# hazdzz/STGCN

Measured on AMD Instinct MI355X. Metric: training windows/sec, METR-LA ChebConv K=3 bs=32, higher is better.
Workload: dtype f32; 1 GPU; C2: METR-LA 207 nodes, STGCNChebGraphConv Ks=3 Kt=3, n_his=12, bs=32 per GPU, fp32, dropout 0.5, AdamW lr 1e-3 wd 1e-3; full step zero_grad+fwd+MSE+bwd+opt; graph=real metr_la adj -> sym_norm_lap -> cheb GSO, global_batch=32, parallelism=dp1, output_block=fused HIP path (stgcn_outblock_*), launch=hipGraph replay, chains=1, backward_products=fp32, operator_products=fp32

## Files before the change

stgcn_amd/csrc/stgcn_capi_bwd.inc:

```

namespace {
int launch_hook_rowstats(const stgcn_ln_hook* hook, const float* dx, long slabs, hipStream_t st) {
    LnBwdArgs hl = zeroed<LnBwdArgs>();
    const LnRowstatOut o = rowstat_out(hook);
    hl.dy = dx; hl.y = o.y; hl.beta = o.beta; hl.gamma = o.gamma; hl.rowstat = o.rowstat;
    hl.n = o.N * o.C; hl.N = o.N; hl.C = o.C; hl.act = o.act; hl.training = o.training; hl.slabs = slabs;
    hl.keep_scale = o.keep_scale; hl.thresh = o.thresh; hl.seed = o.seed; hl.offset = o.offset; hl.offset_dev = o.offset_dev;
    STGCN_LAUNCH_ET("ln_bwd_rowstats", st, (ln_bwd_rowstats_kernel<ET>), dim3(cdiv(hl.slabs * (hl.n / 4), kThreads)), dim3(kThreads), 0, hl);
    return STGCN_OK;
}

struct BlockBwdCall : BlockCall {
    const float* gso_t_pad;
    const float* dy;
    const float* y;
    float* dx;
    const stgcn_ln_hook* dx_hook;
    LnBwdArgs ln;

    int launch_ln_bwd_stats() {
        ln = zeroed<LnBwdArgs>();
        ln.dy = dy; ln.y = y; ln.beta = P->ln_b; ln.U = saved + pl.sv_U2; ln.S = saved + pl.sv_S2; ln.gamma = P->ln_w;
        ln.mean = saved + pl.sv_mean; ln.rstd = saved + pl.sv_rstd; ln.rowstat = reinterpret_cast<float2*>(ws + pl.ws_rowstat_b);
        ln.dZ = ws + pl.ws_dZ2; ln.dgam_part = part() + r.bg.off_ln_g; ln.dbet_part = part() + r.bg.off_ln_b;
        ln.n = d->N * d->c2; ln.N = d->N; ln.C = d->c2; ln.act = d->act; ln.training = training(); ln.spg = r.bg.ln_spg; ln.slabs = r.slabs2;
        ln.keep_scale = keep_scale(); ln.thresh = drop_thresh(d->droprate); ln.seed = seed; ln.offset = offset; ln.offset_dev = offset_dev;
        if (!d->dy_rowstats_ready)
            STGCN_LAUNCH_ET("ln_bwd_rowstats", st, (ln_bwd_rowstats_kernel<ET>), dim3(cdiv(r.slabs2 * (ln.n / 4), kThreads)), dim3(kThreads), 0, ln);
        if (cdiv(ln.n / 4, kThreads) >= kLnBigColgroups) {
            ln.slabconst = reinterpret_cast<float2*>(ws + pl.ws_rowstat_b + 2 * r.rows2);
            STGCN_LAUNCH("ln_slab_consts", st, ln_slab_consts_kernel, dim3((unsigned)r.slabs2), dim3(kThreads), 64, ln);
        }
        return STGCN_OK;
    }
    int launch_ln_gate_bwd() {
        const BwdGeom& bg = r.bg;
        STGCN_LAUNCH("ln_gate_bwd", st, (ln_gate_bwd_kernel<float>), dim3(cdiv(ln.n / 4, kThreads), bg.ln_sg), dim3(kThreads),
                     (8 + 2 * bg.ln_spg) * sizeof(float), ln);
        return STGCN_OK;
    }
    int launch_tc2_bwd() {
        if (g_debug_stages && !g_bf16) {
            const int rc = launch_ln_gate_bwd();
            if (rc) return rc;
        }
        Tc2BwdArgs a = zeroed<Tc2BwdArgs>();
        a.y = hook_mask_from_y() ? y : nullptr;
        a.dy = dy; a.U = ln.U; a.S = ln.S; a.Wp = ws + pl.ws_W2p; a.bias = ws + pl.ws_b2; a.gamma = ln.gamma; a.mean = ln.mean; a.rstd = ln.rstd;
        a.rowstat = ln.rowstat; a.slabconst = ln.slabconst; a.G = saved + pl.sv_G; a.Wd = ws + pl.ws_W2dense; a.dYg = ws + pl.ws_dYg;
        a.part = part() + r.bg.off_k1; a.dgam_part = ln.dgam_part; a.dbet_part = ln.dbet_part;
        a.B = d->B; a.T1 = r.T1; a.T2 = r.T2; a.N = d->N; a.act = d->act; a.training = ln.training; a.node_tiles = r.bg.node_tiles;
        a.keep_scale = ln.keep_scale; a.thresh = ln.thresh; a.seed = seed; a.offset = offset; a.offset_dev = offset_dev;
        const bool recomp = r.tc2_bwd_recompute;
        const int training = ln.training;
        const size_t lds = r.tc2_bwd_lds;
        const dim3 grid((unsigned)r.bg.k1_wgs), blk(512);
#define STGCN_TC2_BWD(C2_, KT_)                                                                                        \
        do {                                                                                                               \
            if (training && d->act == STGCN_ACT_GLU) STGCN_LAUNCH_ETB("tc2_bwd", st, (tc2_bwd_kernel<C2_, KT_, true, 0, RC_, ET>), grid, blk, lds, a);   \
            else if (training) STGCN_LAUNCH_ETB("tc2_bwd", st, (tc2_bwd_kernel<C2_, KT_, true, 1, RC_, ET>), grid, blk, lds, a);      \
            else if (d->act == STGCN_ACT_GLU) STGCN_LAUNCH_ETB("tc2_bwd", st, (tc2_bwd_kernel<C2_, KT_, false, 0, RC_, ET>), grid, blk, lds, a);       \
            else STGCN_LAUNCH_ETB("tc2_bwd", st, (tc2_bwd_kernel<C2_, KT_, false, 1, RC_, ET>), grid, blk, lds, a);                 \
        } while (0)
#define STGCN_TC2_BWD_RC(C2_, KT_) do { if (recomp) { constexpr bool RC_ = true; STGCN_TC2_BWD(C2_, KT_); } else { constexpr bool RC_ = false; STGCN_TC2_BWD(C2_, KT_); } } while (0)
        if (d->Kt == 2) STGCN_TC2_BWD_RC(64, 2); else if (d->Kt == 3) STGCN_TC2_BWD_RC(64, 3); else STGCN_TC2_BWD_RC(64, 4);
#undef STGCN_TC2_BWD_RC
#undef STGCN_TC2_BWD
        return STGCN_OK;
    }
    int launch_staged_tc2_bwd() {
        STGCN_F32_ONLY("ln_gate_bwd + row-tile weight / data gradients of tmp_conv2");
        int rc = launch_ln_gate_bwd();
        if (rc) return rc;
        TconvBwdWeightArgs wa = zeroed<TconvBwdWeightArgs>();
        wa.ts = make_taps(saved + pl.sv_G, d->c1, d->Kt, d->N, r.T1, r.T2, 1, r.rows2);
        wa.dZ = ws + pl.ws_dZ2; wa.part = part() + r.bg.w2.off; wa.NC = r.NC2; wa.Mpad = r.bg.w2.Mpad; wa.rows_per_chunk = r.bg.w2.rows_per_chunk;
        wa.chunks = r.bg.w2.chunks;
        rc = launch_bwd_weight("tconv_bwd_weight.tc2", wa, r.bg.w2, st);
        if (rc) return rc;
        TconvBwdDataArgs a = zeroed<TconvBwdDataArgs>();
        a.ts = make_taps(ws + pl.ws_dZ2, r.NC2, d->Kt, d->N, r.T2, r.T1, -1, r.rows1);
        a.Wp = ws + pl.ws_W2d; a.KCH = d->Kt * r.NC2 / 16; a.Cin = d->c1; a.Gmask = saved + pl.sv_G; a.dX = ws + pl.ws_dYg;
        return launch_bwd_data("tconv_bwd_data.tc2", a, r.CP1 / 16, st);
    }
    int launch_block_gconv_bwd() {
        GconvBwdArgs a = zeroed<GconvBwdArgs>();
        a.dY = ws + pl.ws_dYg; a.X0 = saved + pl.sv_A; a.Xk = saved + pl.sv_Xk; a.LTp = gso_t_pad; a.W = P->gc_w;
        a.dA = ws + pl.ws_dA; a.part = part() + r.bg.off_gc; a.N = d->N; a.NP = r.NP; a.Ks = r.terms;
        a.kipf = d->graph_conv == STGCN_GC_KIPF; a.slabs = r.slabs1;
        a.Gk = r.tiled_gc ? ws + pl.ws_Gk : nullptr; a.tiles_per_wg = r.bg.gc_tiles_per_wg; a.wgs = r.bg.gc_count;
        a.XT = r.tiled_gc && r.terms > 1 ? ws + pl.ws_XT : nullptr;
        return launch_gconv_bwd(a, r.tiled_gc, st);
    }
    int launch_align_gate_bwd() {
        STGCN_F32_ONLY("align_gate_bwd");
        AlignBwdArgs a = zeroed<AlignBwdArgs>();
        a.dA = ws + pl.ws_dA; a.WaT = ws + pl.ws_WaT; a.dZ = ws + pl.ws_dZ1;
        if (r.recompute_tc1) {
            a.Wd = ws + pl.ws_W1dense; a.bias = ws + pl.ws_b1; a.KPd = r.KP1;
            a.ts = input_taps();
        } else {
            a.U = saved + pl.sv_U1; a.S = saved + pl.sv_S1;
        }
        a.part = part() + r.bg.off_al; a.rows = r.rows1; a.c0 = d->c0; a.c1 = d->c1; a.KCH = r.CP1 / 16; a.act = d->act;
        const size_t lds = (size_t)(64 * (d->c1 + 4) + 64 * (d->c0 + 4) + 16 * d->c1) * sizeof(float);
        if (d->c0 == 64) STGCN_LAUNCH("align_gate_bwd", st, (align_gate_bwd_kernel<1>), dim3(r.bg.al_wgs), dim3(kThreads), lds, a);
        else STGCN_LAUNCH("align_gate_bwd", st, (align_gate_bwd_kernel<2>), dim3(r.bg.al_wgs), dim3(kThreads), lds, a);
        return STGCN_OK;
    }
    int launch_tc1_bwd() {
        if (g_debug_stages && !g_bf16) {
            const int rc = launch_align_gate_bwd();
            if (rc) return rc;
        }
        Tc1BwdArgs a = zeroed<Tc1BwdArgs>();
        a.dA = ws + pl.ws_dA; a.U = saved + pl.sv_U1; a.S = saved + pl.sv_S1; a.x = x; a.WaD = ws + pl.ws_WaDense; a.Wd = ws + pl.ws_W1dense;
        a.dx = dx; a.part = part() + r.bg.off_k3; a.B = d->B; a.T = d->T; a.T1 = r.T1; a.N = d->N; a.node_tiles = r.bg.node_tiles;
        const bool hooked = dx_hook && dx_hook->rowstat, epi = hooked && dx_hook->C == d->c_in && dx_hook->N == d->N;
        if (epi) a.rs = rowstat_out(dx_hook);
        const bool x6 = r.tc1_bwd_x6;
        const size_t lds = r.tc1_bwd_lds;
        const dim3 grid((unsigned)r.bg.k3_wgs), blk(768);
#define STGCN_TC1_BWD(CIN_)                                                                                    \
        do {                                                                                                       \
            if (x6 && d->act == STGCN_ACT_GLU) STGCN_LAUNCH("tc1_bwd", st, (tc1_bwd_x6_kernel<64, CIN_, 3, 0>), grid, blk, lds, a);   \
            else if (x6) STGCN_LAUNCH("tc1_bwd", st, (tc1_bwd_x6_kernel<64, CIN_, 3, 1>), grid, blk, lds, a);             \
            else if (d->act == STGCN_ACT_GLU) STGCN_LAUNCH_ETB("tc1_bwd", st, (tc1_bwd_kernel<64, CIN_, 3, 0, ET>), grid, blk, lds, a);   \
            else STGCN_LAUNCH_ETB("tc1_bwd", st, (tc1_bwd_kernel<64, CIN_, 3, 1, ET>), grid, blk, lds, a);             \
        } while (0)
        if (d->c_in == 64) STGCN_TC1_BWD(64); else if (d->c_in == 32) STGCN_TC1_BWD(32); else STGCN_TC1_BWD(16);
#undef STGCN_TC1_BWD
        if (hooked && !epi) return launch_hook_rowstats(dx_hook, dx, (long)d->B * d->T, st);
        return STGCN_OK;
    }
    int launch_thin_bwd() {
        ThinBwdArgs a = zeroed<ThinBwdArgs>();
        a.dA = ws + pl.ws_dA; a.Wd = ws + pl.ws_W1dense; a.bias = ws + pl.ws_b1; a.WaT = ws + pl.ws_WaT;
        a.dZ = d->need_dx ? ws + pl.ws_dZ1 : nullptr; a.part = part() + r.bg.off_al; a.rows = r.rows1; a.c0 = d->c0; a.act = d->act;
        a.ts = input_taps();
        const dim3 grid(r.bg.al_wgs), blk(kThreads);
        if (!r.thin_bwd_waves) {
            const size_t lds = (size_t)(64 * 20 + 64 * (d->c0 + 4) + 64 * (2 * d->c0 + 4) + 64 * 20 + 256) * sizeof(float);
            STGCN_LAUNCH_ETB("align_gate_bwd", st, (thin_tc1_bwd_kernel<ET>), grid, blk, lds, a);
        } else if (d->act == STGCN_ACT_GLU) STGCN_LAUNCH_ETB("align_gate_bwd", st, (thin_tc1_bwd2_kernel<ET, 0>), grid, blk, thin_bwd2_lds_bytes(), a);
        else STGCN_LAUNCH_ETB("align_gate_bwd", st, (thin_tc1_bwd2_kernel<ET, 1>), grid, blk, thin_bwd2_lds_bytes(), a);
        return STGCN_OK;
    }
    int launch_tc1_bwd_weight() {
// ... 63 lines not shown
```

stgcn_amd/csrc/stgcn_kernels_tstep.hip.h:

```cpp
#pragma once
#include <type_traits>
#include "stgcn_device.hip.h"
#include "stgcn_kernels_fwd.hip.h"

namespace stgcn {

struct Tc2BwdArgs {
    const float* y;
    const float* dy;
    const float* U;
    const float* S;
    const float* Wp;
    const float* bias;
    const float* gamma;
    const float* mean;
    const float* rstd;
    const float2* rowstat;
    const float2* slabconst;
    const float* G;
    const float* Wd;
    float* dYg;
    float* part;
    float* dgam_part;
    float* dbet_part;
    int B, T1, T2, N, act, training, node_tiles;
    float keep_scale;
    uint32_t thresh;
    uint64_t seed, offset;
    const uint64_t* offset_dev;
};

constexpr int kTsMaxT = 32;
inline size_t tc2_bwd_lds_bytes(int C2, int Kt, int T1, int T2, bool recomp = true) {
    return ((size_t)(Kt + 1) * 16 * (2 * C2 + 4) + (size_t)T1 * 16 * 20 + 2 * 4 * 16 * 20 + 4 * (size_t)T2 + (recomp ? 2 * 16 * (2 * C2 + 4) : 0)) * sizeof(float);
}

template <int C2, int KT, bool TRAINING, int ACT, bool RECOMP, typename ET>
__global__ __launch_bounds__(512, (C2 == 64 && KT == 3 && ACT == 0 && !RECOMP) ? 4 : 1) void tc2_bwd_kernel(Tc2BwdArgs a) {
    typedef Mma<ET> MM;
    const ET* const dy_ = et_ptr<ET>(a.dy);
    const ET* const ym_ = et_ptr<ET>(a.y ? a.y : a.dy);
    const bool mask_y = TRAINING && a.y != nullptr;
    const ET* const U_ = et_ptr<ET>(a.U);
    const ET* const S_ = et_ptr<ET>(a.S);
    const ET* const G_ = et_ptr<ET>(a.G);
    ET* const dYg_ = et_ptr<ET>(a.dYg);
    constexpr int NC = 2 * C2, LDZ = NC + 4, NTW = NC / 64, QW = NC / 64, IT = C2 / 64, LDG = 20, RING = KT + 1, RED = 4 * 16 * LDG;
    extern __shared__ float stgcn_smem[];
    float* const Zt = stgcn_smem;
    float* const GT = Zt + RING * 16 * LDZ;
    float* const red = GT + a.T1 * 16 * LDG;
    float* const cs = red + 2 * RED;
    float* const USt = cs + 4 * a.T2;
    const bool roleE = threadIdx.x < 256;
    const int tid = threadIdx.x & 255, w = tid >> 6, lane = tid & 63, g = lane >> 4, l15 = lane & 15;
    const int N = a.N, T1 = a.T1, T2 = a.T2;
    const int r = tid >> 4, cq = tid & 15;
    const long items = (long)a.B * a.node_tiles;
    const long it_lo = items * (long)blockIdx.x / (long)gridDim.x, it_hi = items * ((long)blockIdx.x + 1) / (long)gridDim.x;
    float* const part = a.part + (size_t)blockIdx.x * (KT * 16 * NC + NC);
    STGCN_PHASE(8, 0);

    if (roleE) {
        struct Tile { Raw4<ET> dy[IT], u[IT], s[IT], y[IT]; };
        f32x4 dbu[IT], dbq[IT];
#pragma unroll
        for (int it = 0; it < IT; ++it) { dbu[it] = zero4(); dbq[it] = zero4(); }
        const uint64_t off = a.offset + (a.offset_dev ? *a.offset_dev : 0);
        const uint64_t n4 = ((uint64_t)N * C2) >> 2;
        for (long item = it_lo; item < it_hi; ++item) {
        const int b = (int)(item / a.node_tiles), nt = (int)(item - (long)b * a.node_tiles), n0 = nt * 16;
        const bool rv = n0 + r < N;
        const int rc = rv ? n0 + r : N - 1;
        auto fetch = [&](int t2, Tile& t) {
            const size_t e0 = (((size_t)b * T2 + (t2 < T2 ? t2 : T2 - 1)) * N + rc) * C2 + 4 * cq;
#pragma unroll
            for (int it = 0; it < IT; ++it) {
                t.dy[it] = ldraw4(dy_ + e0 + 64 * it);
                if constexpr (TRAINING) t.y[it] = ldraw4(ym_ + e0 + 64 * it);
                if constexpr (!RECOMP) {
                    t.u[it] = ldraw4(U_ + e0 + 64 * it);
                    t.s[it] = ldraw4(S_ + e0 + 64 * it);
                }
            }
        };
        Tile pA, pB;
        fetch(0, pA);
        fetch(1, pB);
        f32x4 gam[IT], dgam[IT], dbet[IT];
#pragma unroll
        for (int it = 0; it < IT; ++it) {
            gam[it] = ld4(a.gamma + (size_t)rc * C2 + 4 * (cq + 16 * it));
            dgam[it] = zero4(); dbet[it] = zero4();
        }
        {
            const int grp = tid >> 5, l32 = tid & 31;
            for (int t0 = 0; t0 < T2; t0 += 8) {
                const int t = t0 + grp;
                const long slab = (long)b * T2 + (t < T2 ? t : 0);
                float x = 0.f, y = 0.f;
                if (a.slabconst) {
                    if (t < T2 && l32 == 0) {
                        const float2 c = a.slabconst[slab];
                        x = c.x; y = c.y;
                    }
                } else {
                    const float2* rs = a.rowstat + slab * N;
                    for (int i0 = 0; i0 < N; i0 += 256) {
                        float2 v[8];
#pragma unroll
                        for (int j = 0; j < 8; ++j) {
                            const int i = i0 + l32 + 32 * j;
                            v[j] = (t < T2 && i < N) ? rs[i] : make_float2(0.f, 0.f);
                        }
#pragma unroll
                        for (int j = 0; j < 8; ++j) {
                            x += v[j].x;
                            y += v[j].y;
                        }
                    }
                }
#pragma unroll
                for (int m = 16; m >= 1; m >>= 1) {
                    x += __shfl_xor(x, m);
                    y += __shfl_xor(y, m);
                }
                if (t < T2 && l32 == 0) {
                    const float inv = a.slabconst ? 1.0f : 1.0f / ((float)N * (float)C2);
                    cs[4 * t] = x * inv;
                    cs[4 * t + 1] = y * inv;
                    cs[4 * t + 2] = a.mean[slab];
                    cs[4 * t + 3] = a.rstd[slab];
                }
            }
        }
        const uint64_t q0 = (((uint64_t)rc * C2) >> 2) + cq;
        auto E = [&](int t, const Tile& tl) {
            float* const Zs = Zt + (t % RING) * 16 * LDZ;
            const float* const Us = USt + (t & 1) * 16 * LDZ + r * LDZ;
            const float c1 = cs[4 * t], c2 = cs[4 * t + 1], mean = cs[4 * t + 2], rstd = cs[4 * t + 3];
#pragma unroll
            for (int it = 0; it < IT; ++it) {
                f32x4 dy = rv ? cvt4(tl.dy[it]) : zero4();
                const int c4 = cq + 16 * it;
                f32x4 u, s;
                if constexpr (RECOMP) {
                    u = ld4(Us + 4 * c4);
                    s = rv ? ld4(Us + C2 + 4 * c4) : zero4();
                } else {
                    u = cvt4(tl.u[it]);
                    s = rv ? cvt4(tl.s[it]) : zero4();
                }
                if constexpr (TRAINING) {
                    if (mask_y) {
                        const f32x4 yv = cvt4(tl.y[it]);
#pragma unroll
                        for (int i = 0; i < 4; ++i) {
                            const float yi = yv[i];
                            dy[i] = drop_kept(yi) ? dy[i] * a.keep_scale : 0.f;
                        }
                    } else {
                        const f32x4 k = dropout_scale4(((uint64_t)b * T2 + t) * n4 + q0 + 16 * it, a.seed, off, a.thresh, a.keep_scale);
#pragma unroll
                        for (int i = 0; i < 4; ++i) dy[i] *= k[i];
                    }
                }
                f32x4 du, dq;
#pragma unroll
                for (int i = 0; i < 4; ++i) {
                    const float xh = (gate_fwd(u[i], s[i], ACT) - mean) * rstd;
                    const float gg = dy[i] * gam[it][i];
                    const float dh = rstd * (gg - c1 - xh * c2);
                    dgam[it][i] += dy[i] * xh;
                    dbet[it][i] += dy[i];
                    float du_, dq_;
                    gate_bwd(dh, u[i], s[i], ACT, du_, dq_);
                    du[i] = du_;
                    dq[i] = dq_;
                }
                dbu[it] += du;
                dbq[it] += dq;
                st4(Zs + r * LDZ + 4 * c4, du);
                st4(Zs + r * LDZ + C2 + 4 * c4, dq);
            }
        };
        __syncthreads();
        if constexpr (RECOMP) __syncthreads();
        STGCN_PHASE(8, 1);
        E(0, pA);
        fetch(2, pA);
        auto stepE = [&](int t1, Tile& ts) __attribute__((always_inline)) {
            __syncthreads();
            if (t1 + 1 < T2) E(t1 + 1, ts);
            fetch(t1 + 3, ts);
        };
        int t1 = 0;
        stepE(t1, pB);
        for (++t1; t1 + 1 < T1; t1 += 2) {
            stepE(t1, pA);
            stepE(t1 + 1, pB);
        }
        if (t1 < T1) stepE(t1, pA);
        STGCN_PHASE(8, 4);
        __syncthreads();
        if (rv) {
#pragma unroll
            for (int it = 0; it < IT; ++it) {
                const size_t o = (size_t)b * N * C2 + (size_t)(n0 + r) * C2 + 4 * (cq + 16 * it);
                st4_wt(a.dgam_part + o, dgam[it]);
                st4_wt(a.dbet_part + o, dbet[it]);
            }
        }
        }
        __syncthreads();
        float* bred = red;
#pragma unroll
        for (int it = 0; it < IT; ++it) {
#pragma unroll
            for (int i = 0; i < 4; ++i) {
                float x = dbu[it][i], y = dbq[it][i];
                x += __shfl_xor(x, 16); y += __shfl_xor(y, 16);
                x += __shfl_xor(x, 32); y += __shfl_xor(y, 32);
                if (g == 0) {
                    bred[w * NC + 4 * (l15 + 16 * it) + i] = x;
                    bred[w * NC + C2 + 4 * (l15 + 16 * it) + i] = y;
                }
            }
        }
        __syncthreads();
        if (tid < NC) part[(size_t)KT * 16 * NC + tid] = (bred[tid] + bred[NC + tid]) + (bred[2 * NC + tid] + bred[3 * NC + tid]);
        STGCN_PHASE(8, 6);
    } else {
        typename MM::frag Wr[KT][QW];
#pragma unroll
        for (int k = 0; k < KT; ++k)
#pragma unroll
            for (int q = 0; q < QW; ++q) Wr[k][q] = MM::cvt(ld4(a.Wd + (size_t)(k * 16 + l15) * NC + w * (NC / 4) + q * 16 + 4 * g));
        constexpr int NTP = C2 / 64, MT = C2 / 16;
        typename MM::frag wP[NTP][KT], wQ[NTP][KT];
        f32x4 bp[NTP], bq[NTP];
        if constexpr (RECOMP) {
#pragma unroll
            for (int j = 0; j < NTP; ++j) {
#pragma unroll
                for (int kc = 0; kc < KT; ++kc) {
                    wP[j][kc] = MM::cvt(ld4(a.Wp + ((size_t)((w + 4 * j) * KT + kc) * 64 + lane) * 4));
                    wQ[j][kc] = MM::cvt(ld4(a.Wp + ((size_t)((w + 4 * j + MT) * KT + kc) * 64 + lane) * 4));
                }
                bp[j] = ld4(a.bias + 16 * (w + 4 * j) + 4 * g);
                bq[j] = ld4(a.bias + C2 + 16 * (w + 4 * j) + 4 * g);
            }
        }
        auto R = [&](int t) __attribute__((always_inline)) {
            float* const Us = USt + (t & 1) * 16 * LDZ + l15 * LDZ;
            typename MM::frag fb[KT];
#pragma unroll
            for (int kc = 0; kc < KT; ++kc) fb[kc] = MM::cvt(gather4(GT + ((t + kc) * 16 + 4 * g) * LDG + l15, LDG));
#pragma unroll
            for (int j = 0; j < NTP; ++j) {
                f32x4 accP = zero4(), accQ = zero4();
#pragma unroll
                for (int kc = 0; kc < KT; ++kc) MM::mma_a2(wP[j][kc], wQ[j][kc], fb[kc], accP, accQ);
                f32x4 u, sg;
#pragma unroll
                for (int e = 0; e < 4; ++e) {
                    u[e] = accP[e] + bp[j][e];
                    sg[e] = sigmoid_f(accQ[e] + bq[j][e]);
                }
                st4(Us + 16 * (w + 4 * j) + 4 * g, u);
                st4(Us + C2 + 16 * (w + 4 * j) + 4 * g, sg);
            }
        };
        f32x4 accw[KT][NTW];
#pragma unroll
        for (int k = 0; k < KT; ++k)
#pragma unroll
            for (int j = 0; j < NTW; ++j) accw[k][j] = zero4();
        for (long item = it_lo; item < it_hi; ++item) {
        const int b = (int)(item / a.node_tiles), nt = (int)(item - (long)b * a.node_tiles), n0 = nt * 16;
        const bool rv = n0 + r < N;
        for (int idx = tid; idx < T1 * 64; idx += 256) {
            const int t = idx >> 6, rem = idx & 63, rr = rem >> 2, q = rem & 3;
            const f32x4 v = n0 + rr < N ? ldx4(G_ + (((size_t)b * T1 + t) * N + n0 + rr) * 16 + 4 * q) : zero4();
#pragma unroll
            for (int i = 0; i < 4; ++i) GT[(t * 16 + 4 * q + i) * LDG + rr] = v[i];
        }
        __syncthreads();
        if constexpr (RECOMP) {
            R(0);
            __syncthreads();
            if (T2 > 1) R(1);
        }
        for (int t1 = 0; t1 < T1; ++t1) {
            __syncthreads();
            if (t1 > 0) {
                const int t = t1 - 1;
                const float* rd = red + (t & 1) * RED;
                float v = (rd[(0 * 16 + r) * LDG + cq] + rd[(1 * 16 + r) * LDG + cq]) + (rd[(2 * 16 + r) * LDG + cq] + rd[(3 * 16 + r) * LDG + cq]);
                if (!(GT[(t * 16 + cq) * LDG + r] > 0.f)) v = 0.f;
                if (rv) stx1(dYg_ + (((size_t)b * T1 + t) * N + n0 + r) * 16 + cq, v);
            }
            if (t1 < T2) {
                const float* const Zs = Zt + (t1 % RING) * 16 * LDZ;
                f32x4 bz[NTW];
#pragma unroll
                for (int s = 0; s < 4; ++s) {
#pragma unroll
                    for (int j = 0; j < NTW; ++j) bz[j][s] = Zs[(4 * g + s) * LDZ + (w * NTW + j) * 16 + l15];
                }
                typename MM::frag fz[NTW];
#pragma unroll
                for (int j = 0; j < NTW; ++j) fz[j] = MM::cvt(bz[j]);
#pragma unroll
                for (int k = 0; k < KT; ++k) {
                    const typename MM::frag af = MM::cvt(ld4(GT + ((t1 + k) * 16 + l15) * LDG + 4 * g));
#pragma unroll
                    for (int j = 0; j < NTW; j += 2) MM::mma_b2(af, fz[j], fz[j + 1], accw[k][j], accw[k][j + 1]);
                }
            }
            f32x4 accd[2] = {zero4(), zero4()};
#pragma unroll
            for (int k = 0; k < KT; ++k) {
                const int ts = t1 - k;
                if (ts >= 0 && ts < T2) {
                    const float* zr = Zt + (ts % RING) * 16 * LDZ + l15 * LDZ + w * (NC / 4) + 4 * g;
#pragma unroll
                    for (int q = 0; q < QW; ++q) {
                        MM::mma_split(Wr[k][q], MM::cvt(ld4(zr + q * 16)), accd[0], accd[1]);
                    }
                }
            }
            st4(red + (t1 & 1) * RED + (w * 16 + l15) * LDG + 4 * g, accd[0] + accd[1]);
            if constexpr (RECOMP) {
                if (t1 + 2 < T2) R(t1 + 2);
            }
        }
        const bool g_last = GT[((T1 - 1) * 16 + cq) * LDG + r] > 0.f;
        __syncthreads();
        {
            const int t = T1 - 1;
            const float* rd = red + (t & 1) * RED;
            float v = (rd[(0 * 16 + r) * LDG + cq] + rd[(1 * 16 + r) * LDG + cq]) + (rd[(2 * 16 + r) * LDG + cq] + rd[(3 * 16 + r) * LDG + cq]);
            if (!g_last) v = 0.f;
            if (rv) stx1(dYg_ + (((size_t)b * T1 + t) * N + n0 + r) * 16 + cq, v);
        }
        }
        STGCN_PHASE(8, 5);
#pragma unroll
        for (int k = 0; k < KT; ++k)
#pragma unroll
            for (int j = 0; j < NTW; ++j)
                st4_wt(part + (size_t)((w * NTW + j) * 16 + l15) * (KT * 16) + k * 16 + 4 * g, accw[k][j]);
        __syncthreads();
        __syncthreads();
    }
}

struct Tc1BwdArgs {
    const float* dA;
    const float* U;
    const float* S;
    const float* x;
    const float* WaD;
    const float* Wd;
    float* dx;
    float* part;
    LnRowstatOut rs;
    int B, T, T1, N, node_tiles;
};
inline size_t tc1_bwd_lds_bytes(int C0, int CIN, int Kt, bool x6 = false) {
    const size_t xt = x6 ? (size_t)(Kt + 1) * 3 * 16 * (CIN + 16) * sizeof(short) : (size_t)(Kt + 1) * CIN * 20 * sizeof(float);
    const size_t zt = x6 ? (size_t)(Kt + 1) * 3 * 16 * (2 * C0 + 8) * sizeof(short) : (size_t)(Kt + 1) * 16 * (2 * C0 + 4) * sizeof(float);
    const size_t rest = ((size_t)(Kt + 1) * 16 * 16 + 2 * 16 * (C0 + 4) + 2 * 16 * (CIN + 4)) * sizeof(float);
    return zt + xt + rest + (x6 ? (size_t)4 * Kt * (2 * C0 / 16) * 64 * 4 * sizeof(short) : 0);
}
inline int tc1_bwd_part_floats(int C0, int CIN, int Kt) { return Kt * CIN * 2 * C0 + 2 * C0 + C0 * 16 + 16; }

__host__ __device__ inline int tc1_bwd_step_weight(int s, int T1, int KT, int CIN) {
    int w = 0;
    if (s < T1) w += KT * (CIN / 16) * 8 + 4;
    for (int k = 0; k < KT; ++k)
        if (s - k >= 0 && s - k < T1) w += 32;
    return w;
}

#define STGCN_TC1BWD_MD_TAP_ASM \
    "ds_read_b128 v[146:149], %[zh] offset:0\n\t" \
    "ds_read_b64 v[144:145], %[zl] offset:0\n\t" \
    "ds_read_b64 v[154:155], %[wl] offset:0\n\t" \
    "ds_read_b128 v[158:161], %[zh] offset:64\n\t" \
    "ds_read_b64 v[156:157], %[zl] offset:32\n\t" \
    "ds_read_b64 v[166:167], %[wl] offset:512\n\t" \
    "s_waitcnt lgkmcnt(3)\n\t" \
    "v_mov_b64 v[150:151], v[146:147]\n\t" \
    "v_mov_b64 v[152:153], %[l0]\n\t" \
    "s_nop 1\n\t" \
    "v_mfma_f32_16x16x32_bf16 %[ca], v[152:155], v[144:147], %[ca]\n\t" \
    "v_mfma_f32_16x16x32_bf16 %[cb], %[w0], v[146:149], %[cb]\n\t" \
    "v_mfma_f32_16x16x32_bf16 %[cc], %[w0], v[148:151], %[cc]\n\t" \
    "ds_read_b128 v[146:149], %[zh] offset:128\n\t" \
    "ds_read_b64 v[144:145], %[zl] offset:64\n\t" \
    "ds_read_b64 v[154:155], %[wl] offset:1024\n\t" \
    "s_waitcnt lgkmcnt(3)\n\t" \
    "v_mov_b64 v[162:163], v[158:159]\n\t" \
    "v_mov_b64 v[164:165], %[l1]\n\t" \
    "s_nop 1\n\t" \
    "v_mfma_f32_16x16x32_bf16 %[ca], v[164:167], v[156:159], %[ca]\n\t" \
    "v_mfma_f32_16x16x32_bf16 %[cb], %[w1], v[158:161], %[cb]\n\t" \
    "v_mfma_f32_16x16x32_bf16 %[cc], %[w1], v[160:163], %[cc]\n\t" \
    "ds_read_b128 v[158:161], %[zh] offset:192\n\t" \
    "ds_read_b64 v[156:157], %[zl] offset:96\n\t" \
    "ds_read_b64 v[166:167], %[wl] offset:1536\n\t" \
    "s_waitcnt lgkmcnt(3)\n\t" \
    "v_mov_b64 v[150:151], v[146:147]\n\t" \
    "v_mov_b64 v[152:153], %[l2]\n\t" \
    "s_nop 1\n\t" \
    "v_mfma_f32_16x16x32_bf16 %[ca], v[152:155], v[144:147], %[ca]\n\t" \
    "v_mfma_f32_16x16x32_bf16 %[cb], %[w2], v[146:149], %[cb]\n\t" \
    "v_mfma_f32_16x16x32_bf16 %[cc], %[w2], v[148:151], %[cc]\n\t" \
    "ds_read_b128 v[146:149], %[zh] offset:256\n\t" \
// ... 1130 lines not shown
```

stgcn_amd/csrc/stgcn_route.h:

```cpp
#pragma once
#include <stdio.h>
#include <stdlib.h>
#include "../../include/stgcn_hip.h"

namespace stgcn {

inline int64_t rup(int64_t v, int64_t m) { return (v + m - 1) / m * m; }
inline int cdiv(int64_t a, int64_t b) { return (int)((a + b - 1) / b); }

inline int env_int(const char* name, int unset) {
    const char* e = getenv(name);
    return e ? atoi(e) : unset;
}
inline bool env_not_zero(const char* name) {
    const char* e = getenv(name);
    return !(e && e[0] == '0');
}
enum FuseBit { FUSE_TC2_BWD = 1, FUSE_TC2_LN_FWD = 2, FUSE_ROWSTATS = 4, FUSE_TC1_BWD = 8, FUSE_TC1_FWD = 16, FUSE_HEAD_LN_FWD = 32, FUSE_HEAD_LN_BWD = 64 };
inline int fuse_mask() { static const int m = env_int("STGCN_FUSE", 0x7fffffff); return m; }
inline bool thin_wave_tiles() { return env_not_zero("STGCN_THIN"); }
inline bool mfma_x6() { return env_not_zero("STGCN_MFMA_X6"); }
inline bool hook_mask_from_y() {
    const char* e = getenv("STGCN_HOOK_MASK");
    return !(e && e[0] == 'p');
// ... 140 lines not shown
    const int colgroups = (int)((n4 + kThreads - 1) / kThreads);
    int sg = (512 + colgroups - 1) / colgroups;
    if (colgroups >= kLnBigColgroups) sg = (4096 + colgroups - 1) / colgroups;
    if (sg > slabs2) sg = (int)slabs2;
    if (sg < 1) sg = 1;
    g.ln_spg = (int)((slabs2 + sg - 1) / sg);
    g.ln_sg = (int)((slabs2 + g.ln_spg - 1) / g.ln_spg);
    g.k1 = tc2_bwd_fused_ok(c1, c2, Kt, T1, T2) ? 1 : 0;
    g.node_tiles = (N + 15) / 16;
    {
        const long items = (long)B * g.node_tiles, cap = 2L * device_cus();
        g.k1_wgs = (int)(items < cap ? items : cap);
    }
    g.k1_stride = Kt * 16 * 2 * c2 + 2 * c2;
    if (g.k1) {
        g.ln_spg = T2;
        g.ln_sg = B;
    }
    const long tiles1 = (rows1 + kTileRows - 1) / kTileRows;
    g.thin = (Kt * c_in <= 4 && c0 == 64 && c1 == 16) ? 1 : 0;
    const int al_cap = g.thin ? (rows1 >= (1L << 18) && thin_wave_tiles() ? 768 : 512) : 1024;
    g.al_wgs = (int)(tiles1 < al_cap ? tiles1 : al_cap);
    long o = 0;
    auto take = [&](long f) { long at = o; o += (f + 63) / 64 * 64; return at; };
    g.off_ln_g = take((long)g.ln_sg * n);
    g.off_ln_b = take((long)g.ln_sg * n);
    g.gc_stride = (terms + 1) * 256;
    g.gc_count = (int)slabs1;
    g.gc_tiles_per_wg = 0;
    if (gc_is_tiled(N, terms)) {
        const long tiles16 = (rows1 + 15) / 16;
        long per = (tiles16 + 1023) / 1024;
        per = (per + 3) / 4 * 4;
        g.gc_tiles_per_wg = (int)per;
        g.gc_count = (int)((tiles16 + per - 1) / per);
    }
    g.off_gc = take((long)g.gc_count * g.gc_stride);
    g.al_stride = c0 * c1 + c1 + (g.thin ? 16 * 2 * c0 + 2 * c0 : 0);
    g.off_al = take((long)g.al_wgs * g.al_stride);
    g.w1 = wgrad_geom(rows1, Kt * c_in, 2 * c0, 0);
    g.w1.off = take(g.w1.floats);
    g.w2 = wgrad_geom(rows2, Kt * c1, 2 * c2, 0);
    g.w2.off = take(g.k1 ? 0 : g.w2.floats);
    g.off_k1 = take(g.k1 ? (long)g.k1_wgs * g.k1_stride : 0);
    g.k3 = (need_dx && !g.thin && tc1_bwd_shape_ok(c_in, c0, c1, Kt)) ? 1 : 0;
    g.k3_wgs = tc1_range_wgs((long)B * g.node_tiles, T, 1);
    g.k3_stride = tc1_bwd_part_floats(c0, c_in, Kt);
    g.off_k3 = take(g.k3 ? (long)g.k3_wgs * g.k3_stride : 0);
    g.total = o;
    return g;
}

inline int thin_fwd_wgs(int64_t rows) {
    constexpr int tpw = 2;
    const int64_t tiles = (rows + 15) / 16, want = (tiles + 4 * tpw - 1) / (4 * tpw), cap = 4L * device_cus();
    return (int)(want < 1 ? 1 : want < cap ? want : cap);
}

enum Tc1FwdForm { TC1_FWD_TSTEP, TC1_FWD_THIN, TC1_FWD_ROWTILE };
enum BwdForm { BWD_FUSED, BWD_THIN, BWD_STAGED };

struct BlockRoute {
    int T1, T2, NP, KP1, KP2, NC1, NC2, CP_in, CP1, terms;
    int64_t rows0, rows1, rows2, slabs1, slabs2;
    bool bf16;
    bool recompute_tc1;
    bool thin;
    bool dense_W1;
    bool dense_Wa;
    bool dense_Wa_slot;
    bool dense_W2;
    Tc1FwdForm tc1_fwd;
    bool tc1_fwd_x6;
    int tc1_fwd_wgs;
    size_t tc1_fwd_lds;
    bool tc2_ln_fused;
    bool tc2_ln_x6;
    int tc2_ln_tpw, tc2_ln_groups, tc2_ln_peers, tc2_ln_threads;
    size_t tc2_ln_lds;
    bool stored_US2;
    BwdGeom bg;
    BwdForm tc2_bwd;
    bool tc2_bwd_recompute;
    size_t tc2_bwd_lds;
    BwdForm tc1_bwd;
    bool thin_bwd_waves;
    bool tc1_bwd_x6;
    size_t tc1_bwd_lds;
    bool tiled_gc;
    bool bf16_bwd_ok;
};

inline bool bf16_backward_ok(BwdForm tc2_bwd, BwdForm tc1_bwd, int need_dx) {
    return tc2_bwd == BWD_FUSED && (tc1_bwd == BWD_FUSED || (tc1_bwd == BWD_THIN && !need_dx));
}

inline BlockRoute route_block(const stgcn_stblock_desc* d) {
    BlockRoute r;
    r.T1 = d->T - d->Kt + 1;
    r.T2 = r.T1 - d->Kt + 1;
    r.terms = d->graph_conv == STGCN_GC_KIPF ? 2 : d->Ks;
    r.tiled_gc = gc_is_tiled(d->N, r.terms);
    r.NP = gc_padded_nodes(d->N, r.terms);
    r.KP1 = (int)rup((int64_t)d->Kt * d->c_in, 16);
    r.KP2 = (int)rup((int64_t)d->Kt * d->c1, 16);
    r.NC1 = 2 * d->c0;
    r.NC2 = 2 * d->c2;
    r.CP_in = (int)rup(d->c_in, 16);
    r.CP1 = (int)rup(d->c1, 16);
    r.rows0 = (int64_t)d->B * d->T * d->N;
    r.rows1 = (int64_t)d->B * r.T1 * d->N;
    r.rows2 = (int64_t)d->B * r.T2 * d->N;
    r.slabs1 = (int64_t)d->B * r.T1;
    r.slabs2 = (int64_t)d->B * r.T2;
    r.bf16 = d->dtype == STGCN_DTYPE_BF16;
    r.bg = bwd_geom(d->B, d->T, d->N, d->c_in, d->c0, d->c1, d->c2, d->Kt, r.terms, d->need_dx);
    const bool x6 = mfma_x6() && !r.bf16;
    const bool tc1_fwd_ok = tc1_fwd_shape_ok(d->c_in, d->c0, d->c1, d->Kt), tc1_bwd_ok = tc1_bwd_shape_ok(d->c_in, d->c0, d->c1, d->Kt);
    const bool tc1_ts = (tc1_bwd_ok || tc1_fwd_ok) && d->Kt * d->c_in > 4;
    r.recompute_tc1 = d->Kt * d->c_in <= 16;
    r.thin = r.bg.thin;
    r.dense_W1 = r.recompute_tc1 || tc1_ts;
    r.dense_Wa = tc1_ts && !r.thin;
    r.dense_Wa_slot = tc1_ts || r.thin;
    r.dense_W2 = r.bg.k1;
    if (!r.recompute_tc1 && !d->x_bstride && !d->x_index_dev && tc1_fwd_ok) r.tc1_fwd = TC1_FWD_TSTEP;
    else if (r.thin && thin_wave_tiles()) r.tc1_fwd = TC1_FWD_THIN;
    else r.tc1_fwd = TC1_FWD_ROWTILE;
    r.tc1_fwd_x6 = x6;
    r.tc1_fwd_lds = tc1_fwd_lds_bytes(d->c_in, d->Kt, x6);
    r.tc1_fwd_wgs = tc1_range_wgs((long)d->B * r.bg.node_tiles, r.T1, r.bf16 ? 2 : 1);
    r.tc2_ln_fused = tc2_ln_fwd_fused_ok(d->c1, d->c2, d->Kt, d->N);
    r.tc2_ln_peers = tc2_ln_peers(d->N, r.slabs2);
    const bool wide = d->N <= (r.bf16 ? 384 : 256) && r.slabs2 <= 2L * device_cus();
    r.tc2_ln_x6 = x6 && d->N <= 256 && r.slabs2 <= 2L * device_cus() && d->Kt <= 3;
    if (r.tc2_ln_peers == 2) r.tc2_ln_tpw = d->N <= 256 ? 2 : 3;
    else if (r.tc2_ln_peers == 4) r.tc2_ln_tpw = d->N <= 256 ? 1 : 2;
    else if (wide) r.tc2_ln_tpw = d->N <= 256 ? 4 : 6;
    else r.tc2_ln_tpw = d->N <= 224 ? 7 : 14;
    r.tc2_ln_groups = r.tc2_ln_tpw >= 7 ? 2 : 4;
    r.tc2_ln_threads = r.tc2_ln_groups * 256;
    r.tc2_ln_lds = tc2_ln_fwd_lds_bytes(d->Kt, d->N, r.tc2_ln_x6);
    r.tc2_bwd = r.bg.k1 ? BWD_FUSED : BWD_STAGED;
    r.tc2_bwd_recompute = tc2_recompute(r.bf16);
    r.tc2_bwd_lds = tc2_bwd_lds_bytes(d->c2, d->Kt, r.T1, r.T2, r.tc2_bwd_recompute);
    r.stored_US2 = !r.tc2_ln_fused || !r.bg.k1 || g_debug_stages || !r.tc2_bwd_recompute;
    r.tc1_bwd = r.bg.k3 ? BWD_FUSED : r.thin ? BWD_THIN : BWD_STAGED;
    r.thin_bwd_waves = thin_wave_tiles();
    r.tc1_bwd_x6 = x6 && g_bwd_precision == 0 && tc1_bwd_lds_bytes(d->c0, d->c_in, d->Kt, true) <= 160 * 1024;
    r.tc1_bwd_lds = tc1_bwd_lds_bytes(d->c0, d->c_in, d->Kt, r.tc1_bwd_x6);
    r.bf16_bwd_ok = bf16_backward_ok(r.tc2_bwd, r.tc1_bwd, d->need_dx);
    return r;
}

}
```

Before: 91470 windows/s.

## Add bf16x6 split-product MFMA path for tmp_conv2 fused backward kernel

Adds an X6 variant of the fused tc2 backward kernel that stores the gate-gradient tile and G inputs in LDS as three-way bf16 splits (hi/mid/lo). It then computes the weight-gradient and data-gradient products with 16x16x32 bf16 MFMAs in a six-product form that approximates fp32 accuracy. The aim is to replace slower fp32 matrix ops and halve LDS footprint per element so four waves-per-SIMD occupancy applies for the GLU and non-GLU cases. The cost is extra split and convert work, more MFMA issues, and scheduling barriers. The path is gated on the x6 route flag, fp32 backward precision, no recompute, c2=64, Kt=3, and an LDS budget.

```diff
diff --git a/stgcn_amd/csrc/stgcn_capi_bwd.inc b/stgcn_amd/csrc/stgcn_capi_bwd.inc
--- a/stgcn_amd/csrc/stgcn_capi_bwd.inc
+++ b/stgcn_amd/csrc/stgcn_capi_bwd.inc
@@ -63,7 +63,16 @@
             else STGCN_LAUNCH_ETB("tc2_bwd", st, (tc2_bwd_kernel<C2_, KT_, false, 1, RC_, ET>), grid, blk, lds, a);                 \
         } while (0)
 #define STGCN_TC2_BWD_RC(C2_, KT_) do { if (recomp) { constexpr bool RC_ = true; STGCN_TC2_BWD(C2_, KT_); } else { constexpr bool RC_ = false; STGCN_TC2_BWD(C2_, KT_); } } while (0)
-        if (d->Kt == 2) STGCN_TC2_BWD_RC(64, 2); else if (d->Kt == 3) STGCN_TC2_BWD_RC(64, 3); else STGCN_TC2_BWD_RC(64, 4);
+#define STGCN_TC2_BWD_X6(C2_, KT_)                                                                                     \
+        do {                                                                                                               \
+            if (training && d->act == STGCN_ACT_GLU) STGCN_LAUNCH("tc2_bwd", st, (tc2_bwd_kernel<C2_, KT_, true, 0, false, float, true>), grid, blk, lds, a);   \
+            else if (training) STGCN_LAUNCH("tc2_bwd", st, (tc2_bwd_kernel<C2_, KT_, true, 1, false, float, true>), grid, blk, lds, a);      \
+            else if (d->act == STGCN_ACT_GLU) STGCN_LAUNCH("tc2_bwd", st, (tc2_bwd_kernel<C2_, KT_, false, 0, false, float, true>), grid, blk, lds, a);       \
+            else STGCN_LAUNCH("tc2_bwd", st, (tc2_bwd_kernel<C2_, KT_, false, 1, false, float, true>), grid, blk, lds, a);                 \
+        } while (0)
+        if (r.tc2_bwd_x6) STGCN_TC2_BWD_X6(64, 3);
+        else if (d->Kt == 2) STGCN_TC2_BWD_RC(64, 2); else if (d->Kt == 3) STGCN_TC2_BWD_RC(64, 3); else STGCN_TC2_BWD_RC(64, 4);
+#undef STGCN_TC2_BWD_X6
 #undef STGCN_TC2_BWD_RC
 #undef STGCN_TC2_BWD
         return STGCN_OK;
diff --git a/stgcn_amd/csrc/stgcn_kernels_tstep.hip.h b/stgcn_amd/csrc/stgcn_kernels_tstep.hip.h
--- a/stgcn_amd/csrc/stgcn_kernels_tstep.hip.h
+++ b/stgcn_amd/csrc/stgcn_kernels_tstep.hip.h
@@ -31,12 +31,24 @@
 };
 
 constexpr int kTsMaxT = 32;
-inline size_t tc2_bwd_lds_bytes(int C2, int Kt, int T1, int T2, bool recomp = true) {
+inline size_t tc2_bwd_lds_bytes(int C2, int Kt, int T1, int T2, bool recomp = true, bool x6 = false) {
+    if (x6) return ((size_t)(Kt + 1) * 3 * 16 * (2 * C2 + 16) + (size_t)T1 * 3 * 16 * 16) * sizeof(short) + ((size_t)2 * 4 * 16 * 20 + 4 * (size_t)T2) * sizeof(float);
     return ((size_t)(Kt + 1) * 16 * (2 * C2 + 4) + (size_t)T1 * 16 * 20 + 2 * 4 * 16 * 20 + 4 * (size_t)T2 + (recomp ? 2 * 16 * (2 * C2 + 4) : 0)) * sizeof(float);
 }
 
-template <int C2, int KT, bool TRAINING, int ACT, bool RECOMP, typename ET>
-__global__ __launch_bounds__(512, (C2 == 64 && KT == 3 && ACT == 0 && !RECOMP) ? 4 : 1) void tc2_bwd_kernel(Tc2BwdArgs a) {
+#if defined(__HIP_DEVICE_COMPILE__)
+#define STGCN_SCHED_FENCE() __builtin_amdgcn_sched_barrier(0)
+#else
+#define STGCN_SCHED_FENCE() ((void)0)
+#endif
+#if defined(__HIP_DEVICE_COMPILE__)
+#define STGCN_OPAQUE(x) asm volatile("" : "+v"(x))
+#else
+#define STGCN_OPAQUE(x) ((void)0)
+#endif
+template <int C2, int KT, bool TRAINING, int ACT, bool RECOMP, typename ET, bool X6 = false>
+__global__ __launch_bounds__(512, (C2 == 64 && KT == 3 && (ACT == 0 || X6) && !RECOMP) ? 4 : 1) void tc2_bwd_kernel(Tc2BwdArgs a) {
+    static_assert(!X6 || (!RECOMP && std::is_same<ET, float>::value), "bf16x6 is a product form of the fp32 blocks, which read the stored gate inputs");
     typedef Mma<ET> MM;
     const ET* const dy_ = et_ptr<ET>(a.dy);
     const ET* const ym_ = et_ptr<ET>(a.y ? a.y : a.dy);
@@ -48,8 +60,11 @@
     constexpr int NC = 2 * C2, LDZ = NC + 4, NTW = NC / 64, QW = NC / 64, IT = C2 / 64, LDG = 20, RING = KT + 1, RED = 4 * 16 * LDG;
     extern __shared__ float stgcn_smem[];
     float* const Zt = stgcn_smem;
-    float* const GT = Zt + RING * 16 * LDZ;
-    float* const red = GT + a.T1 * 16 * LDG;
+    constexpr int LDZP = NC + 16, ZPL = 16 * LDZP, ZSLOT = 3 * ZPL, GPL = 16 * 16, GSLOT = 3 * GPL;
+    float* const GT = Zt + (X6 ? RING * ZSLOT / 2 : RING * 16 * LDZ);
+    float* const red = GT + (X6 ? a.T1 * GSLOT / 2 : a.T1 * 16 * LDG);
+    short* const Zh = reinterpret_cast<short*>(Zt);
+    short* const Gh = reinterpret_cast<short*>(GT);
     float* const cs = red + 2 * RED;
     float* const USt = cs + 4 * a.T2;
     const bool roleE = threadIdx.x < 256;
@@ -70,6 +85,9 @@
         const uint64_t n4 = ((uint64_t)N * C2) >> 2;
         for (long item = it_lo; item < it_hi; ++item) {
         const int b = (int)(item / a.node_tiles), nt = (int)(item - (long)b * a.node_tiles), n0 = nt * 16;
+        int te = tid;
+        if constexpr (X6) STGCN_OPAQUE(te);
+        const int r = te >> 4, cq = te & 15;
         const bool rv = n0 + r < N;
         const int rc = rv ? n0 + r : N - 1;
         auto fetch = [&](int t2, Tile& t) {
@@ -180,8 +198,17 @@
                 }
                 dbu[it] += du;
                 dbq[it] += dq;
-                st4(Zs + r * LDZ + 4 * c4, du);
-                st4(Zs + r * LDZ + C2 + 4 * c4, dq);
+                if constexpr (X6) {
+                    short* const Zp = Zh + (size_t)(t % RING) * ZSLOT + r * LDZP + 4 * c4;
+                    STGCN_SCHED_FENCE();
+                    st_frag3(Zp, ZPL, split3(du));
+                    STGCN_SCHED_FENCE();
+                    st_frag3(Zp + C2, ZPL, split3(dq));
+                    STGCN_SCHED_FENCE();
+                } else {
+                    st4(Zs + r * LDZ + 4 * c4, du);
+                    st4(Zs + r * LDZ + C2 + 4 * c4, dq);
+                }
             }
         };
         __syncthreads();
@@ -214,6 +241,9 @@
         }
         __syncthreads();
         float* bred = red;
+        int tb = tid;
+        if constexpr (X6) STGCN_OPAQUE(tb);
+        const int w = tb >> 6, g = (tb >> 4) & 3, l15 = tb & 15;
 #pragma unroll
         for (int it = 0; it < IT; ++it) {
 #pragma unroll
@@ -228,14 +258,28 @@
             }
         }
         __syncthreads();
-        if (tid < NC) part[(size_t)KT * 16 * NC + tid] = (bred[tid] + bred[NC + tid]) + (bred[2 * NC + tid] + bred[3 * NC + tid]);
+        float* const part_e = X6 ? a.part + (size_t)blockIdx.x * (KT * 16 * NC + NC) + tb : part + tb;
+        if (tb < NC) part_e[(size_t)KT * 16 * NC] = (bred[tb] + bred[NC + tb]) + (bred[2 * NC + tb] + bred[3 * NC + tb]);
         STGCN_PHASE(8, 6);
     } else {
-        typename MM::frag Wr[KT][QW];
-#pragma unroll
-        for (int k = 0; k < KT; ++k)
-#pragma unroll
-            for (int q = 0; q < QW; ++q) Wr[k][q] = MM::cvt(ld4(a.Wd + (size_t)(k * 16 + l15) * NC + w * (NC / 4) + q * 16 + 4 * g));
+        typename MM::frag Wr[X6 ? 1 : KT][X6 ? 1 : QW];
+        bf16x8 Whh[X6 ? KT : 1], Wmm[X6 ? KT : 1], Wll[X6 ? KT : 1];
+        static_assert(!X6 || QW == 2, "two 16-channel fragments per wave and tap");
+#pragma unroll
+        for (int k = 0; k < KT; ++k) {
+            f32x4 wv[QW];
+#pragma unroll
+            for (int q = 0; q < QW; ++q) wv[q] = ld4(a.Wd + (size_t)(k * 16 + l15) * NC + w * (NC / 4) + q * 16 + 4 * g);
+            if constexpr (X6) {
+                const Frag3 f0 = split3(wv[0]), f1 = split3(wv[QW - 1]);
+                Whh[k] = cat8(f0.h, f1.h);
+                Wmm[k] = cat8(f0.m, f1.m);
+                Wll[k] = cat8(f0.l, f1.l);
+            } else {
+#pragma unroll
+                for (int q = 0; q < QW; ++q) Wr[k][q] = MM::cvt(wv[q]);
+            }
+        }
         constexpr int NTP = C2 / 64, MT = C2 / 16;
         typename MM::frag wP[NTP][KT], wQ[NTP][KT];
         f32x4 bp[NTP], bq[NTP];
@@ -282,8 +326,12 @@
         for (int idx = tid; idx < T1 * 64; idx += 256) {
             const int t = idx >> 6, rem = idx & 63, rr = rem >> 2, q = rem & 3;
             const f32x4 v = n0 + rr < N ? ldx4(G_ + (((size_t)b * T1 + t) * N + n0 + rr) * 16 + 4 * q) : zero4();
-#pragma unroll
-            for (int i = 0; i < 4; ++i) GT[(t * 16 + 4 * q + i) * LDG + rr] = v[i];
+            if constexpr (X6) {
+                st_frag3(Gh + (size_t)t * GSLOT + rr * 16 + 4 * q, GPL, split3(v));
+            } else {
+#pragma unroll
+                for (int i = 0; i < 4; ++i) GT[(t * 16 + 4 * q + i) * LDG + rr] = v[i];
+            }
         }
         __syncthreads();
         if constexpr (RECOMP) {
@@ -291,16 +339,49 @@
             __syncthreads();
             if (T2 > 1) R(1);
         }
+        auto g_pos = [&](int t, int r, int cq) __attribute__((always_inline)) {
+            if constexpr (X6) {
+                const short h = Gh[(size_t)t * GSLOT + r * 16 + cq];
+                return h > 0 && h <= (short)0x7f80;
+            } else {
+                return GT[(t * 16 + cq) * LDG + r] > 0.f;
+            }
+        };
         for (int t1 = 0; t1 < T1; ++t1) {
             __syncthreads();
             if (t1 > 0) {
                 const int t = t1 - 1;
+                int tf = tid;
+                if constexpr (X6) STGCN_OPAQUE(tf);
+                const int r = tf >> 4, cq = tf & 15;
                 const float* rd = red + (t & 1) * RED;
                 float v = (rd[(0 * 16 + r) * LDG + cq] + rd[(1 * 16 + r) * LDG + cq]) + (rd[(2 * 16 + r) * LDG + cq] + rd[(3 * 16 + r) * LDG + cq]);
-                if (!(GT[(t * 16 + cq) * LDG + r] > 0.f)) v = 0.f;
-                if (rv) stx1(dYg_ + (((size_t)b * T1 + t) * N + n0 + r) * 16 + cq, v);
-            }
-            if (t1 < T2) {
+                if (!g_pos(t, r, cq)) v = 0.f;
+                if (n0 + r < N) stx1(dYg_ + (((size_t)b * T1 + t) * N + n0 + r) * 16 + cq, v);
+            }
+            int tm = tid;
+            if constexpr (X6) STGCN_OPAQUE(tm);
+            const int w = tm >> 6, g = (tm >> 4) & 3, l15 = tm & 15;
+            if constexpr (X6) {
+              if (t1 < T2) {
+                const short* const Zp = Zh + (size_t)(t1 % RING) * ZSLOT + (w * NTW) * 16;
+#pragma unroll
+                for (int j = 0; j < NTW; ++j) {
+                    const s16x4 zh = ld_tr4(Zp + j * 16, LDZP, g, l15), zm = ld_tr4(Zp + ZPL + j * 16, LDZP, g, l15), zl = ld_tr4(Zp + 2 * ZPL + j * 16, LDZP, g, l15);
+                    const bf16x8 zlh = cat8(zl, zh), zhm = cat8(zh, zm), zmh = cat8(zm, zh);
+#pragma unroll
+                    for (int k = 0; k < KT; ++k) {
+                        const short* const gp = Gh + (size_t)(t1 + k) * GSLOT;
+                        const s16x4 ah = ld_tr4(gp, 16, g, l15), am = ld_tr4(gp + GPL, 16, g, l15), al = ld_tr4(gp + 2 * GPL, 16, g, l15);
+                        const bf16x8 ahl = cat8(ah, al), amh = cat8(am, ah);
+                        accw[k][j] = __builtin_amdgcn_mfma_f32_16x16x32_bf16(ahl, zlh, accw[k][j], 0, 0, 0);
+                        accw[k][j] = __builtin_amdgcn_mfma_f32_16x16x32_bf16(amh, zhm, accw[k][j], 0, 0, 0);
+                        accw[k][j] = __builtin_amdgcn_mfma_f32_16x16x32_bf16(amh, zmh, accw[k][j], 0, 0, 0);
+                        STGCN_SCHED_FENCE();
+                    }
+                }
+              }
+            } else if (t1 < T2) {
                 const float* const Zs = Zt + (t1 % RING) * 16 * LDZ;
                 f32x4 bz[NTW];
 #pragma unroll
@@ -319,23 +400,39 @@
                 }
             }
             f32x4 accd[2] = {zero4(), zero4()};
+            f32x4 accs = zero4();
 #pragma unroll
             for (int k = 0; k < KT; ++k) {
                 const int ts = t1 - k;
                 if (ts >= 0 && ts < T2) {
+                  if constexpr (X6) {
+                    const short* const zr = Zh + (size_t)(ts % RING) * ZSLOT + l15 * LDZP + w * (NC / 4) + 4 * g;
+                    const bf16x8 zhh = cat8(*reinterpret_cast<const s16x4*>(zr), *reinterpret_cast<const s16x4*>(zr + 16));
+                    const bf16x8 zmm = cat8(*reinterpret_cast<const s16x4*>(zr + ZPL), *reinterpret_cast<const s16x4*>(zr + ZPL + 16));
+                    const bf16x8 zll = cat8(*reinterpret_cast<const s16x4*>(zr + 2 * ZPL), *reinterpret_cast<const s16x4*>(zr + 2 * ZPL + 16));
+                    accs = __builtin_amdgcn_mfma_f32_16x16x32_bf16(Whh[k], zll, accs, 0, 0, 0);
+                    accs = __builtin_amdgcn_mfma_f32_16x16x32_bf16(Wll[k], zhh, accs, 0, 0, 0);
+                    accd[k & 1] = __builtin_amdgcn_mfma_f32_16x16x32_bf16(Whh[k], zhh, accd[k & 1], 0, 0, 0);
+                    accs = __builtin_amdgcn_mfma_f32_16x16x32_bf16(Wmm[k], zmm, accs, 0, 0, 0);
+                    accs = __builtin_amdgcn_mfma_f32_16x16x32_bf16(Whh[k], zmm, accs, 0, 0, 0);
+                    accs = __builtin_amdgcn_mfma_f32_16x16x32_bf16(Wmm[k], zhh, accs, 0, 0, 0);
+                    STGCN_SCHED_FENCE();
+                  } else {
                     const float* zr = Zt + (ts % RING) * 16 * LDZ + l15 * LDZ + w * (NC / 4) + 4 * g;
 #pragma unroll
                     for (int q = 0; q < QW; ++q) {
                         MM::mma_split(Wr[k][q], MM::cvt(ld4(zr + q * 16)), accd[0], accd[1]);
                     }
-                }
-            }
+                  }
+                }
+            }
+            if constexpr (X6) accd[1] += accs;
             st4(red + (t1 & 1) * RED + (w * 16 + l15) * LDG + 4 * g, accd[0] + accd[1]);
             if constexpr (RECOMP) {
                 if (t1 + 2 < T2) R(t1 + 2);
             }
         }
-        const bool g_last = GT[((T1 - 1) * 16 + cq) * LDG + r] > 0.f;
+        const bool g_last = g_pos(T1 - 1, r, cq);
         __syncthreads();
         {
             const int t = T1 - 1;
diff --git a/stgcn_amd/csrc/stgcn_route.h b/stgcn_amd/csrc/stgcn_route.h
--- a/stgcn_amd/csrc/stgcn_route.h
+++ b/stgcn_amd/csrc/stgcn_route.h
@@ -246,6 +246,7 @@
     BwdGeom bg;
     BwdForm tc2_bwd;
     bool tc2_bwd_recompute;
+    bool tc2_bwd_x6;
     size_t tc2_bwd_lds;
     BwdForm tc1_bwd;
     bool thin_bwd_waves;
@@ -307,7 +308,9 @@
     r.tc2_ln_lds = tc2_ln_fwd_lds_bytes(d->Kt, d->N, r.tc2_ln_x6);
     r.tc2_bwd = r.bg.k1 ? BWD_FUSED : BWD_STAGED;
     r.tc2_bwd_recompute = tc2_recompute(r.bf16);
-    r.tc2_bwd_lds = tc2_bwd_lds_bytes(d->c2, d->Kt, r.T1, r.T2, r.tc2_bwd_recompute);
+    r.tc2_bwd_x6 = x6 && g_bwd_precision == 0 && !r.tc2_bwd_recompute && d->c2 == 64 && d->Kt == 3 &&
+                   tc2_bwd_lds_bytes(d->c2, d->Kt, r.T1, r.T2, false, true) <= 80 * 1024;
+    r.tc2_bwd_lds = tc2_bwd_lds_bytes(d->c2, d->Kt, r.T1, r.T2, r.tc2_bwd_recompute, r.tc2_bwd_x6);
     r.stored_US2 = !r.tc2_ln_fused || !r.bg.k1 || g_debug_stages || !r.tc2_bwd_recompute;
     r.tc1_bwd = r.bg.k3 ? BWD_FUSED : r.thin ? BWD_THIN : BWD_STAGED;
     r.thin_bwd_waves = thin_wave_tiles();
```

Result: slower. 90290 windows/s (-1.3%).
